# EsauPR/3d-pose-baseline

Measured on AMD Instinct MI355X. Metric: poses/sec at batch 64 (H3.6M 16-joint), higher is better.
Workload: dtype f32; 1 GPU; cfg2 inference: L=1024, 2 residual blocks, BN(eval), keep=1; a step = one batch-64 request (its own 64 poses); 86 requests per persistent p3d_serve launch (5504 rows, whole network per XCD); global_batch=64, linear_size=1024, num_layers=2, parallelism=dp1

## Files before the change

3d-pose-baseline_amd/csrc/p3d.hip:

```cpp
#include <hip/hip_ext.h>
#include "p3d_kernels.h"
#include "p3d_bf16.h"
#include "p3d_eval.h"
#include "p3d_gemm.h"
#include "p3d_data.h"
#include "p3d_clip.h"
#include "p3d_serve.h"
#include "p3d_serve6.h"
#include "p3d_serve_plan.h"
#include "p3d_gemv.h"
#include "p3d_xchg.h"
#include "../../include/p3d.h"

#include <math.h>
#include <stdlib.h>
#include <stdio.h>
#include <string.h>

#include <cstdlib>
#include <mutex>
#include <string>
#include <unordered_set>
#include <vector>

// ... 1074 lines not shown
  }
  if (training) {
    m->serve_ec_dirty = true;
    m->have_cache = true;
    m->x_cached = x;
    m->B_cached = B;
    m->keep = keep_prob;
    m->seed = seed; m->ctr = ctr; m->row_off = row_offset;
    m->ctr_dev = (ctr == P3D_CTR_GLOBAL_STEP) ? &m->dstate->global_step : nullptr;
  }
  return P3D_OK;
}

extern "C" int p3d_forward(p3d_model* m, const float* x, int64_t B, float* y, int32_t training,
                           float keep_prob, uint64_t seed, uint64_t ctr, int64_t row_offset, void* stream) {
  return p3d_forward_ex(m, x, B, y, training, keep_prob, seed, ctr, row_offset, 0, stream);
}

static_assert(kServe6Rows == P3D_SERVE6_ROWS, "p3d_serve_plan.h plans for the slabs p3d_serve.h sizes");
#define SERVE_KERNEL_k_serve(D, NDT, NCM, RT, PAIR) k_serve<D, NDT, 4>
#define SERVE_KERNEL_k_serve5(D, NDT, NCM, RT, PAIR) k_serve5<D, NDT, 2, 2>
#define SERVE_KERNEL_k_serve6(D, NDT, NCM, RT, PAIR) k_serve6<D, NDT, NCM, RT, PAIR>
#define SERVE_KERNEL_k_serve6_rounds(D, NDT, NCM, RT, PAIR) k_serve6_rounds<D, NDT, NCM, RT>
#define SERVE_KERNEL_ROW(KIND, D, NDT, NCM, RT, PAIR) SERVE_KERNEL_##KIND(D, NDT, NCM, RT, PAIR),
static void (*const kServeKernels[])(ServeArgs) = {P3D_SERVE_FORMS(SERVE_KERNEL_ROW)};
#undef SERVE_KERNEL_ROW

#define SERVE_TRY(expr)                                                                                     \
  do {                                                                                                      \
    hipError_t e_ = (expr);                                                                                 \
    if (e_ != hipSuccess) return fail(P3D_ERR_HIP, std::string("p3d_serve: ") + hipGetErrorString(e_)); \
  } while (0)

static const char* serve_shape_error(const p3d_cfg& c, int64_t B) {
  if (B <= 0) return "p3d_serve: batch must be positive";
  if (c.dtype != P3D_DTYPE_F32) return "p3d_serve: fp32 models only";
  if (c.linear_size <= 0 || c.linear_size % 128 != 0 || c.input_size > 64 || c.output_size > 64 ||
      2 * c.num_layers + 2 > P3D_SERVE_MAXL)
    return "p3d_serve: needs linear_size % 128 == 0, input/output size <= 64, <= 7 blocks";
  if ((B + 63) / 64 > 0x7fffffff) return "p3d_serve: too many rows";
  return nullptr;
}

static int serve_alloc(p3d_model* m) {
  const p3d_cfg& c = m->cfg;
  const int L = c.linear_size, U = L / 32, NDT = (c.output_size + 15) / 16;
// ... 49 lines not shown
  a.sync = m->serve_sync; a.err = m->serve_err;
  a.epoch = m->serve_sync + 3 * P3D_SERVE_SYNC_WORDS;
  a.census_extra = m->serve_fault ? 1 : 0;
  a.delay = (m->serve_delay > 0 && (m->serve_calls++ & 1) == 0) ? m->serve_delay : 0;
  a.delay_xcc = m->serve_delay_xcc;
  a.max_groups = m->serve_groups;
  for (size_t l = 0; l < m->layers.size(); ++l) {
    const Layer& ly = m->layers[l];
    ServeLayer& s = a.ly[l];
    s.Wf = m->wpk + ly.wf; s.bias = m->flat[0] + ly.b;
    if (ly.bn) {
      s.gamma = m->flat[0] + ly.gamma; s.beta = m->flat[0] + ly.beta;
      s.mmean = m->moving + ly.mmean; s.mvar = m->moving + ly.mvar;
    }
    s.wsq = c.max_norm ? m->wsq + ly.widx : nullptr;
  }
  if (B != m->serve_B || (t != nullptr) != m->serve_with_loss) {
    const ServeChoice ch = serve_plan(L, c.num_layers, (c.output_size + 15) / 16, m->serve_grid, m->serve_knobs, B,
                                      t != nullptr);
    if (ch.refused) return fail(P3D_ERR_ARG, ch.refused);
    m->serve_choice = ch; m->serve_B = B; m->serve_with_loss = t != nullptr;
  }
  const ServeForm& f = *m->serve_choice.form;
  const bool use6 = f.kind == SK_k_serve6 || f.kind == SK_k_serve6_rounds;
  a.split = m->serve_choice.S;
  a.nb = m->serve_choice.nb;
  a.ecg = m->serve_ecg;
  HP(0);
  hipStreamCaptureStatus cap = hipStreamCaptureStatusNone;
  SERVE_TRY(hipStreamIsCapturing(st, &cap));
  const bool capturing = cap != hipStreamCaptureStatusNone;
  HP(1);

  if (use6 && (m->serve_ec_dirty || capturing)) {
    const int nl = 2 * c.num_layers + 1;
    k_serve_prep<<<(unsigned)((nl * L + 255) / 256), 256, 0, st>>>(a, m->serve_ecg);
    LAUNCH_CHECK("k_serve_prep");
    if (!capturing) m->serve_ec_dirty = false;
  }
  if (use6) {
    a.act = m->serve6_act;
    a.part = nullptr;
  } else {
    a.sync = m->serve_sync + 2 * P3D_SERVE_SYNC_WORDS;
    SERVE_TRY(hipMemsetAsync(a.sync, 0, P3D_SERVE_SYNC_WORDS * sizeof(unsigned), st));
  }
  if (t) {
    a.tgt = t; a.loss = loss;
    a.lpart = m->serve_loss; a.lcnt = (unsigned*)(m->serve_loss + kServeLossTiles);
    if (m->hwait && !f.pair) { a.hflag = m->hflag_dev; a.hseq = m->hwait; m->harmed = true; }
  }
  ProfScope ps(m, "serve");
  HP(2);
  go(ps, kServeKernels[&f - kServeForms], dim3((unsigned)m->serve_grid), dim3(f.kind == SK_k_serve ? 512 : 256), st, a);
  HP(3);
  LAUNCH_CHECK("k_serve");
  return P3D_OK;
}
#undef SERVE_TRY

extern "C" int p3d_serve(p3d_model* m, const float* x, int64_t B, float* y, void* stream) {
  return serve_impl(m, x, B, y, nullptr, nullptr, stream);
}

extern "C" int p3d_serve_mse(p3d_model* m, const float* x, int64_t B, float* y, const float* t, float* loss,
                             void* stream) {
  if (!t || !loss) return fail(P3D_ERR_ARG, "p3d_serve_mse: null argument");
  return serve_impl(m, x, B, y, t, loss, stream);
}

extern "C" int p3d_serve_plan(const p3d_cfg* cfg, int32_t cus, int64_t B, int32_t with_loss, char* name,
                              int64_t name_len, int32_t* shape) {
  if (!cfg || !name || name_len <= 0 || cus < 1) return fail(P3D_ERR_ARG, "p3d_serve_plan: bad argument");
  if (const char* why = serve_shape_error(*cfg, B)) return fail(P3D_ERR_ARG, why);
  const ServeChoice ch = serve_plan(cfg->linear_size, cfg->num_layers, (cfg->output_size + 15) / 16, cus,
                                    serve_knobs_from_env(), B, with_loss != 0);
  if (ch.refused) return fail(P3D_ERR_ARG, ch.refused);
// ... 1071 lines not shown
```

3d-pose-baseline_amd/csrc/p3d_serve6.h:

```cpp
#pragma once
#include "p3d_serve.h"

#ifndef P3D_S6_PIN_ARGS
#define P3D_S6_PIN_ARGS 1
#endif
#ifndef P3D_S6_COMBINE_BATCH
#define P3D_S6_COMBINE_BATCH 1
#endif
#ifndef P3D_S6_OUT_PRE
#define P3D_S6_OUT_PRE 1
#endif
#ifndef P3D_S6_LATE_EPOCH
#define P3D_S6_LATE_EPOCH 1
#endif


#ifdef P3D_TRACE
#define P3D_S6_STAMP(row, k)                                                              \
  do {                                                                                    \
    if (tr6 && (row) && threadIdx.x == 0) {                                               \
      tr6[(k)] = wall_clock64();                                                          \
      tr6[64 + (k)] = __builtin_amdgcn_s_memtime();                                       \
    }                                                                                     \
  } while (0)
#else
#define P3D_S6_STAMP(row, k) do { } while (0)
#endif

__global__ __launch_bounds__(256) void k_serve_prep(ServeArgs p, float* ecg) {
  const int i = blockIdx.x * 256 + threadIdx.x;
  const int L = p.L, nl = 2 * p.nblk + 1;
  if (i >= nl * L) return;
  const int l = i / L, col = i % L, t = col >> 4, j = col & 15;
  const ServeLayer& ly = p.ly[l];
  float inv = 1.f, shift = 0.f;
  if (p.bn) {
    inv = (1.0f / sqrtf(ly.mvar[col] + p.eps)) * ly.gamma[col];
    shift = ly.beta[col] - ly.mmean[col] * inv;
  }
  float* e = ecg + ((int64_t)l * (L >> 4) + t) * 48;
  e[j] = ly.bias[col]; e[16 + j] = inv; e[32 + j] = shift;
  if (col == 0)
    ecg[(int64_t)nl * (L >> 4) * 48 + l] = ly.wsq ? fmaxf(sqrtf(*ly.wsq), 1.0f) : 1.0f;
}

__device__ __forceinline__ int p3d_tile_owner(int t, int n, int T) { return ((t + 1) * n - 1) / T; }

template <int DEPTH, int NDT, int NCM, int RT = 4, bool PAIR = false>
__global__ __launch_bounds__(256) __attribute__((amdgpu_waves_per_eu(1, 1))) void k_serve6(ServeArgs p) {
  constexpr bool ROUNDS = false;
#include "p3d_serve6_body.h"
}

template <int DEPTH, int NDT, int NCM, int RT>
__global__ __launch_bounds__(256) __attribute__((amdgpu_waves_per_eu(1, 1))) void k_serve6_rounds(ServeArgs p) {
  constexpr bool PAIR = true, ROUNDS = true;
#include "p3d_serve6_body.h"
}
```

3d-pose-baseline_amd/csrc/p3d_serve6_body.h:

```cpp
  static_assert(RT >= 1 && RT <= 16, "row tiles per unit");
  static_assert(!PAIR || (NCM == 2 && DEPTH == 4), "the pair form: 2 column tiles per member, a 4-deep ring");
  constexpr int ROWS = 16 * RT;
  constexpr int UMAX = (RT * NCM + 3) / 4;
  constexpr int OCH = RT * NCM < 4 ? RT * NCM : 4;
#ifndef P3D_S6_DA
  constexpr int DA = PAIR ? DEPTH : RT >= 6 ? (DEPTH >= 8 ? 4 : 2) : (NCM >= 7 && DEPTH > 2 ? 2 : DEPTH);
#else
  constexpr int DA = RT >= 6 ? P3D_S6_DA : (NCM >= 7 && DEPTH > 2 ? 2 : DEPTH);
#endif
#ifndef P3D_S6_PD
  constexpr int PD = NCM <= 4 ? 2 : 1;
#else
  constexpr int PD = P3D_S6_PD;
#endif
  static_assert(!PAIR || DA == DEPTH, "the pair form's ring runs on across blocks: every slot holds both operands");
  __shared__ __attribute__((aligned(16))) f32x4 red[(PAIR ? 2 : 1) * 4 * RT * NCM * 64];
  constexpr int ECT = NCM >= 7 ? NCM : 2 * NCM;
  __shared__ __attribute__((aligned(16))) float ec[(P3D_SERVE_MAXL - 1) * ECT * 48];
  __shared__ float ecm[P3D_SERVE_MAXL];
  __shared__ int sh[32];
  const int tid = threadIdx.x, lane = tid & 63, w = __builtin_amdgcn_readfirstlane(tid >> 6);
#if P3D_S6_PIN_ARGS
  asm volatile("" ::"s"(p.split), "s"(p.delay), "s"(p.delay_xcc), "s"(p.census_extra), "s"(p.max_groups),
               "s"(p.nb), "s"(p.L), "s"(p.K0), "s"(p.nblk), "s"(p.M), "s"(p.x), "s"(p.epoch), "s"(p.ecg),
               "s"(p.err), "s"(p.sync), "s"(p.act), "s"(p.ly[0].Wf), "s"(gridDim.x));
#endif
  const int L = p.L, ngL = L >> 4, T = ngL, ngK0 = p.K0 >> 4;
  const int q4 = 4 * (lane >> 4);
  const int S = min(max(p.split, 1), 8);
#ifdef P3D_TRACE
  const unsigned long long t_start = wall_clock64();
  unsigned long long* tr6 = nullptr;
#endif

  const int nxg = (int)(gridDim.x >> 3);
  unsigned xr;
  asm volatile("s_getreg_b32 %0, hwreg(HW_REG_XCC_ID)" : "=s"(xr));
  const int xcc = (int)(xr & 7u), rx = (int)(blockIdx.x >> 3);
  unsigned ep = 0;
  if (tid == 0) {
    if (p.delay > 0 && xcc == p.delay_xcc)
      for (int i = 0; i < p.delay; ++i) __builtin_amdgcn_s_sleep(127);
    const bool bad = (gridDim.x & 7u) != 0u || p.split < 1 || p.split > 8 || p.census_extra;
    sh[0] = (int)(((unsigned)xcc - blockIdx.x) & 7u);
    sh[2] = bad ? 1 : 0;
    sh[4] = 0;
    sh[5] = -1;
    sh[6] = 0;
    if (bad) __hip_atomic_store(p.err, 1, __ATOMIC_RELAXED, __HIP_MEMORY_SCOPE_SYSTEM);
  }
  const int nl_ec = 2 * p.nblk + 1, tot_ec = nl_ec * ECT * 48;
  constexpr int ECN = ((P3D_SERVE_MAXL - 1) * ECT * 48 + 255) / 256;
  auto place = [&](auto cnt, int xcc, int rx, int& r, int& n, int& gid, int& gi, int& ng) {
    const int half = rx % S;
    r = rx / S;
    n = (cnt(xcc) + S - 1 - half) / S;
    gid = xcc * S + half;
    ng = 0;
    gi = 0;
    for (int h = 0; h < S; ++h)
#pragma unroll
      for (int x = 0; x < 8; ++x) {
        const int c = (cnt(x) + S - 1 - h) / S;
        if (c > 0) { if (x == xcc && h == half) gi = ng; ++ng; }
      }
    if (p.max_groups > 0 && ng > p.max_groups) {
      ng = p.max_groups;
      if (gi >= ng) gi = p.nb;
    }
    if ((T + n - 1) / n > ECT) gi = -1;
    if (PAIR && ((T + n - 1) / n > NCM || n > T || (T >> 2) < 3 * DEPTH)) gi = -1;
// ... 5 lines not shown
#pragma unroll
    for (int j = 0; j < (PAIR ? 0 : UMAX); ++j) {
      const int u = min(w + 4 * j, RT * NCM - 1), rt = u / NCM, cc = u % NCM;
      int64_t rowc = (int64_t)gi_ * ROWS + 16 * rt + (lane & 15);
      rowc = rowc < p.M ? (rowc > 0 ? rowc : 0) : p.M - 1;
      const int t = min(max(tlo + (cc < nck ? cc : nck - 1), 0), T - 1);
#pragma unroll
      for (int g = 0; g < 2; ++g) {
        const int gg = min(g, ngK0 - 1);
        xa0[j][g] = *(const f32x4*)(p.x + rowc * p.K0 + 16 * gg + q4);
        wb0[j][g] = *(const f32x4*)(p.ly[0].Wf + ((int64_t)(t * ngK0 + gg) * 64 + lane) * 4);
      }
      if (ngK0 > 2) {
#pragma unroll
        for (int g = 2; g < 4; ++g) {
          const int gg = min(g, ngK0 - 1);
          xa0[j][g] = *(const f32x4*)(p.x + rowc * p.K0 + 16 * gg + q4);
          wb0[j][g] = *(const f32x4*)(p.ly[0].Wf + ((int64_t)(t * ngK0 + gg) * 64 + lane) * 4);
        }
      }
    }
#pragma unroll
    for (int k = 0; k < ECN; ++k) {
      const int idx = tid + 256 * k, idc = idx < tot_ec ? idx : 0;
      const int l = idc / (ECT * 48), rem = idc % (ECT * 48), cs = rem / 48, j = rem % 48;
      const float e = p.ecg[((int64_t)l * T + min(tlo + cs, T - 1)) * 48 + j];
      vec[k] = idx < tot_ec ? e : 0.f;
    }
    const float e = p.ecg[(int64_t)nl_ec * T * 48 + (tid < nl_ec ? tid : 0)];
    wq = tid < nl_ec ? e : 1.f;
  };
  int r, n, gid, gi, ng;
  const bool placeable = (gridDim.x & 7u) == 0u && p.split >= 1 && p.split <= 8;
  place([&](int) { return nxg; }, xcc, rx, r, n, gid, gi, ng);
#if P3D_S6_LATE_EPOCH
  prefetch(gi, (T * r) / n, (T * (r + 1)) / n);
  if (tid == 0 && placeable) ep = __hip_atomic_load(p.epoch + gid, __ATOMIC_RELAXED, __HIP_MEMORY_SCOPE_AGENT);
#else
  if (tid == 0 && placeable) ep = __hip_atomic_load(p.epoch + gid, __ATOMIC_RELAXED, __HIP_MEMORY_SCOPE_AGENT);
  prefetch(gi, (T * r) / n, (T * (r + 1)) / n);
  if (tid == 0) {
    sh[3] = (int)(ep & 1u);
    sh[5] = (placeable && r == 0 && gi >= 0 && gi < p.nb) ? gid : -1;
  }
  __syncthreads();
#endif
#ifdef P3D_TRACE
// ... 49 lines not shown
      const int u = min(w + 4 * j, RT * NCM - 1), rt = u / NCM, cc = u % NCM;
      int64_t rowc = rbase + 16 * rt + (lane & 15);
      rowc = rowc < p.M ? rowc : p.M - 1;
      const int t = c0 + (cc < nck ? cc : nck - 1);
#pragma unroll
      for (int g = 0; g < 2; ++g) {
        const int gg = min(g, ngK0 - 1);
        xa[j][g] = *(const f32x4*)(p.x + rowc * p.K0 + 16 * gg + q4);
        wb[j][g] = *(const f32x4*)(li.Wf + ((int64_t)(t * ngK0 + gg) * 64 + lane) * 4);
      }
      if (ngK0 > 2) {
#pragma unroll
        for (int g = 2; g < 4; ++g) {
          const int gg = min(g, ngK0 - 1);
          xa[j][g] = *(const f32x4*)(p.x + rowc * p.K0 + 16 * gg + q4);
          wb[j][g] = *(const f32x4*)(li.Wf + ((int64_t)(t * ngK0 + gg) * 64 + lane) * 4);
        }
      }
    }
  };
  {
#pragma unroll
    for (int k = 0; k < ECN; ++k)
      if (tid + 256 * k < tot_ec) ec[tid + 256 * k] = vec[k];
    if (tid < nl_ec) ecm[tid] = wq;
    __syncthreads();
  }
  P3D_S6_STAMP(trs, 4);
  auto epi_c = [&](const f32x4& b4, const f32x4& inv4, const f32x4& sh4, f32x4 acc) -> f32x4 {
    f32x4 o;
#pragma unroll
    for (int k = 0; k < 4; ++k) {
      const float z = acc[k] + b4[k];
      o[k] = p3d_relu(p.bn ? z * inv4[k] + sh4[k] : z);
    }
    return o;
  };
  auto epi_t = [&](int l, int cs, f32x4 acc) -> f32x4 {
    const float* e = ec + (l * ECT + cs) * 48 + q4;
    return epi_c(*(const f32x4*)e, *(const f32x4*)(e + 16), *(const f32x4*)(e + 32), acc);
  };
  auto maxnorm_div = [&](int l, f32x4& acc) {
    const float mx = ecm[l];
#pragma unroll
    for (int k = 0; k < 4; ++k) acc[k] = acc[k] / mx;
  };

// ... 73 lines not shown
    }
  };

  const float qnan = __builtin_nanf("");
  constexpr int OGH = 8;
  f32x4 ow0[OGH], ow1[OGH];
  auto out_wpre = [&]() {
    const int oo = (((PAIR ? 2 : 1) * RT * NDT * r) / n) % NDT;
    const __amdgpu_buffer_rsrc_t r4 = p3d_rsrc(lo.Wf);
#pragma unroll
    for (int g = 0; g < OGH; ++g) {
      ow0[g] = __builtin_bit_cast(f32x4, __builtin_amdgcn_raw_buffer_load_b128(r4, ((oo * ngL + gb + min(g, gcount - 1)) * 64 + lane) * 16, 0, 0));
      ow1[g] = __builtin_bit_cast(f32x4, __builtin_amdgcn_raw_buffer_load_b128(r4, ((oo * ngL + gb + min(OGH + g, gcount - 1)) * 64 + lane) * 16, 0, 0));
    }
  };
#ifdef P3D_TRACE
#define P3D_S6_OSTAMP(k)                                                                               \
  do {                                                                                                 \
    if (tid == 0 && blockIdx.x < 1024) g_p3d_trace[21504 + blockIdx.x * 4 + (k)] = wall_clock64();     \
  } while (0)
#else
#define P3D_S6_OSTAMP(k) do { } while (0)
#endif
  auto out_phase = [&](int64_t orow0, int64_t orow1, bool pre) {
    constexpr int OT = RT * NDT, OTT = PAIR ? 2 * OT : OT;
    const int o_lo = (OTT * r) / n, o_hi = (OTT * (r + 1)) / n;
    P3D_S6_OSTAMP(0);
    const __amdgpu_buffer_rsrc_t ryA = p3d_rsrc(act + 3 * slab), r4 = p3d_rsrc(lo.Wf);
    const __amdgpu_buffer_rsrc_t ryB = p3d_rsrc(act + (PAIR ? 7 : 3) * slab);
    for (int c0 = o_lo; c0 < o_hi; c0 += OCH) {
      const int nt = min(OCH, o_hi - c0);
      f32x4 tv = f32x4{0.f, 0.f, 0.f, 0.f};
      if (p.tgt && w < nt) {
        const bool tb = PAIR && c0 + w >= OT;
        tv = p3d_serve_load_tgt<NDT>(p, (tb ? c0 + w - OT : c0 + w) * 64 + lane, tb ? orow1 : orow0);
      }
      f32x4 oacc[OCH];
#pragma unroll
      for (int j = 0; j < OCH; ++j) oacc[j] = f32x4{0.f, 0.f, 0.f, 0.f};
#pragma unroll
      for (int j = 0; j < OCH; ++j) {
        if (j >= nt) break;
        const bool tb = PAIR && c0 + j >= OT;
        const int tile = tb ? c0 + j - OT : c0 + j, ort = tile / NDT, oo = tile % NDT;
        const __amdgpu_buffer_rsrc_t ry = tb ? ryB : ryA;
        constexpr int GH = OGH;
        auto ld_half = [&](int gs, f32x4 (&av)[GH], f32x4 (&wv)[GH], bool wpre) {
#pragma unroll
          for (int g = 0; g < GH; ++g) {
            const int gg = gb + min(gs + g, gcount - 1);
            av[g] = p3d_ld_sc1(ry, ((ort * ngL + gg) * 64 + lane) * 16);
            if (!wpre)
              wv[g] = __builtin_bit_cast(f32x4, __builtin_amdgcn_raw_buffer_load_b128(r4, ((oo * ngL + gg) * 64 + lane) * 16, 0, 0));
          }
        };
        auto mma_half = [&](int gs, const f32x4 (&av)[GH], const f32x4 (&wv)[GH]) {
#pragma unroll
          for (int g = 0; g < GH; ++g) {
            if (gs + g >= gcount) break;
#pragma unroll
            for (int e = 0; e < 4; ++e) oacc[j] = __builtin_amdgcn_mfma_f32_16x16x4f32(av[g][e], wv[g][e], oacc[j], 0, 0, 0);
          }
        };
        for (int g0 = 0; g0 < gcount; g0 += 2 * GH) {
          f32x4 a0[GH], w0[GH], a1[GH], w1[GH];
          const bool wpre = P3D_S6_OUT_PRE && pre && c0 == o_lo && j == 0 && g0 == 0;
          if (wpre) {
#pragma unroll
            for (int g = 0; g < GH; ++g) { w0[g] = ow0[g]; w1[g] = ow1[g]; }
          }
          ld_half(g0, a0, w0, wpre);
          ld_half(g0 + GH, a1, w1, wpre);
          mma_half(g0, a0, w0);
          mma_half(g0 + GH, a1, w1);
        }
      }
#pragma unroll
      for (int j = 0; j < OCH; ++j)
        if (j < nt) red[(w * OCH + j) * 64 + lane] = oacc[j];
      if (c0 == o_lo) P3D_S6_OSTAMP(1);
      __syncthreads();
      if (w < nt) {
        f32x4 sl[4];
#pragma unroll
        for (int k = 0; k < 4; ++k) sl[k] = red[(k * OCH + w) * 64 + lane];
        __builtin_amdgcn_sched_barrier(0);
        f32x4 tot = sl[0];
#pragma unroll
        for (int k = 1; k < 4; ++k) tot += sl[k];
        if (broken) tot = f32x4{qnan, qnan, qnan, qnan};
        const bool tb = PAIR && c0 + w >= OT;
        const int tile = tb ? c0 + w - OT : c0 + w;
        const int64_t orow = tb ? orow1 : orow0;
        const float se = p3d_serve_store_out<NDT>(p, lo, tot, tile * 64 + lane, orow, tv);
        if (p.tgt)
          p3d_serve_loss_tile<!PAIR>(p, se, (orow >> 4) * NDT + tile, ((p.M + 15) >> 4) * NDT);
      }
      if (c0 == o_lo) P3D_S6_OSTAMP(2);
      __syncthreads();
    }
  };

  f32x4 rbp[PD][NCM];
  auto b_prefetch = [&](int layer, int c0) {
    const int nck = min(NCM, t_hi - c0);
#pragma unroll
    for (int cc = 0; cc < NCM; ++cc) {
      const int t = c0 + (cc < nck ? cc : nck - 1);
      const f32x4* pbn = (const f32x4*)p.ly[layer].Wf + ((int64_t)t * ngL + gb) * 64 + lane;
#pragma unroll
      for (int d = 0; d < PD; ++d) rbp[d][cc] = pbn[d * 64];
    }
  };

  if constexpr (!PAIR) {
  int c0b = 0;
  if (gi < p.nb) {
    if (t_lo < t_hi) in_compute(t_lo, xa0, wb0, act);
    P3D_S6_STAMP(trs, 5);
    in_layer((int64_t)gi * ROWS, act, t_lo + NCM);
    P3D_S6_STAMP(trs, 2);
    if (t_lo < t_hi) b_prefetch(1, t_lo);
// ... 216 lines not shown
  const int aoff0 = (gb * 64 + lane) * 16, rstride = ngL * 1024, voff = lane * 16;
  int toff[NCM];
#pragma unroll
  for (int cc = 0; cc < NCM; ++cc) toff[cc] = ((t_lo + (cc < nck ? cc : nck - 1)) * ngL + gb) * 1024;
  f32x4 ra_[DA][RT], rb_[DEPTH][NCM];
  auto ring_load = [&](int layer, const float* A) {
    const __amdgpu_buffer_rsrc_t ra = p3d_rsrc(A), rw = p3d_rsrc(p.ly[layer].Wf);
#pragma unroll
    for (int d = 0; d < DEPTH; ++d) {
      if (d < DA)
#pragma unroll
        for (int t = 0; t < RT; ++t) ra_[d][t] = p3d_ld_sc1(ra, aoff0 + t * rstride + d * 1024);
#pragma unroll
      for (int cc = 0; cc < NCM; ++cc)
        rb_[d][cc] = __builtin_bit_cast(f32x4, __builtin_amdgcn_raw_buffer_load_b128(rw, voff, toff[cc] + d * 1024, 0));
      __builtin_amdgcn_sched_barrier(0);
    }
  };
  int rot = 0;
  int64_t orowA = 0, orowB = 0;
#ifdef P3D_TRACE
  int rnd = 0;
#endif
  if constexpr (ROUNDS) {
    if (gi < p.nb) {
      const int64_t rowA = (int64_t)gi * ROWS, rowB = (int64_t)(gi + ng) * ROWS;
      {
        f32x4 xa[UMAX][4], wa[UMAX][4], xb[UMAX][4], wbb[UMAX][4];
        in_issue(rowA, t_lo, xa, wa);
        in_issue(rowB, t_lo, xb, wbb);
        in_compute(t_lo, xa, wa, act);
        P3D_S6_STAMP(trs, 5);
        group_sync(false, false);
        in_compute(t_lo, xb, wbb, act + 4 * slab);
        P3D_S6_STAMP(trs, 2);
      }
      wait_for(nsync);
      P3D_S6_STAMP(trs, 3);
      {
        const float *A0, *r0;
        float* Y0;
        slabs(0, 0, A0, Y0, r0);
        ring_load(1, A0);
      }
    }
  }
// ... 180 lines not shown
    if (tid == 0 && blockIdx.x < 1024) g_p3d_trace[20480 + blockIdx.x] = wall_clock64();
#endif
    trs = false;
    if constexpr (ROUNDS) {
      rot = rotn;
      orowA = rowA;
      orowB = rowB;
#ifdef P3D_TRACE
      ++rnd;
#endif
    }
  }
  if constexpr (ROUNDS) {
    if (gi < p.nb) {
      const int64_t rowA = orowA, rowB = orowB;
      asm volatile("s_waitcnt vmcnt(0)" ::: "memory");
      post_wave();
      if (P3D_S6_OUT_PRE) out_wpre();
      wait_for(nsync);
      out_phase(rowA, rowB, true);
    }
  }
  }
  if (tid == 0 && sh[5] >= 0)
    __hip_atomic_fetch_add(p.epoch + sh[5], 1u, __ATOMIC_RELAXED, __HIP_MEMORY_SCOPE_AGENT);
  }
```

3d-pose-baseline_amd/csrc/p3d_serve_plan.h:

```cpp
#pragma once
#include <algorithm>
#include <cstdint>
#include <cstdlib>
#include <string>

#define P3D_SERVE_FORMS(X)                                                                      \
  X(k_serve, 2, 1, 0, 4, false) X(k_serve, 2, 2, 0, 4, false) X(k_serve, 2, 3, 0, 4, false)      \
  X(k_serve, 2, 4, 0, 4, false)                                                                 \
  X(k_serve5, 4, 1, 0, 4, false) X(k_serve5, 4, 2, 0, 4, false) X(k_serve5, 4, 3, 0, 4, false)  \
  X(k_serve5, 4, 4, 0, 4, false)                                                                \
  X(k_serve5, 2, 1, 0, 4, false) X(k_serve5, 2, 2, 0, 4, false) X(k_serve5, 2, 3, 0, 4, false)  \
  X(k_serve5, 2, 4, 0, 4, false)                                                                \
  X(k_serve6, 4, 3, 2, 4, false) X(k_serve6, 2, 3, 2, 4, false) X(k_serve6, 4, 3, 4, 4, false)  \
  X(k_serve6, 2, 3, 4, 4, false) X(k_serve6, 4, 3, 7, 4, false) X(k_serve6, 2, 3, 7, 4, false)  \
  X(k_serve6, 2, 3, 8, 4, false)                                                                \
  X(k_serve6, 4, 3, 2, 1, false) X(k_serve6, 4, 3, 2, 2, false) X(k_serve6, 2, 3, 11, 2, false) \
  X(k_serve6, 4, 3, 2, 6, false) X(k_serve6, 4, 3, 2, 8, false) X(k_serve6, 4, 3, 2, 10, false) \
  X(k_serve6, 4, 3, 2, 12, false) X(k_serve6, 4, 3, 2, 16, false)                               \
  X(k_serve6, 4, 3, 2, 5, true) X(k_serve6_rounds, 4, 3, 2, 5, true)

enum ServeKind { SK_k_serve, SK_k_serve5, SK_k_serve6, SK_k_serve6_rounds };

struct ServeForm {
  ServeKind kind;
  int depth, ndt, ncm, rt;
  bool pair;
};

#define P3D_SERVE_FORM_ROW(KIND, DEPTH, NDT, NCM, RT, PAIR) {SK_##KIND, DEPTH, NDT, NCM, RT, PAIR},
constexpr ServeForm kServeForms[] = {P3D_SERVE_FORMS(P3D_SERVE_FORM_ROW)};
#undef P3D_SERVE_FORM_ROW

inline const ServeForm* serve_form_find(ServeKind kind, int depth, int ndt, int ncm, int rt, bool pair) {
  for (const ServeForm& f : kServeForms)
    if (f.kind == kind && f.depth == depth && f.ndt == ndt && f.ncm == ncm && f.rt == rt && f.pair == pair) return &f;
  return nullptr;
}

inline std::string serve_kernel_name(ServeKind kind, int depth, int ndt, int ncm, int rt, bool pair) {
  const std::string dn = std::to_string(depth) + ", " + std::to_string(ndt);
  const std::string cr = ", " + std::to_string(ncm) + ", " + std::to_string(rt);
  switch (kind) {
    case SK_k_serve: return "k_serve<" + dn + ", 4>";
    case SK_k_serve5: return "k_serve5<" + dn + ", 2, 2>";
    case SK_k_serve6_rounds: return "k_serve6_rounds<" + dn + cr + ">";
    default: return "k_serve6<" + dn + cr + (pair ? ", true>" : ">");
  }
}
inline std::string serve_form_name(const ServeForm& f) {
  return serve_kernel_name(f.kind, f.depth, f.ndt, f.ncm, f.rt, f.pair);
}

inline ServeKind serve_fallback_kind(int num_layers) { return num_layers > 0 ? SK_k_serve5 : SK_k_serve; }
inline int serve_fallback_depth(int L, int num_layers) { return num_layers > 0 && (L / 64) % 4 == 0 ? 4 : 2; }

constexpr int kServe6Rows = 4096;
constexpr int64_t kServeLossTiles = kServe6Rows / 16 * 4;

struct ServeKnobs {
  int serve6 = 1;
  int max_nb = 32;
  int split = 0;
  int rt = 0;
  int depth = 2;
  int pair = 1;
  int rounds = 1;
};

inline ServeKnobs serve_knobs_from_env() {
  ServeKnobs k;
  const auto read = [](const char* name, int& v) { if (const char* ev = getenv(name)) v = atoi(ev); };
  read("P3D_SERVE6", k.serve6);
  read("P3D_SERVE6_MAX_NB", k.max_nb);
  read("P3D_SERVE6_SPLIT", k.split);
  read("P3D_SERVE6_RT", k.rt);
  read("P3D_SERVE6_DEPTH", k.depth);
  read("P3D_SERVE6_PAIR", k.pair);
  read("P3D_SERVE6_ROUNDS", k.rounds);
  return k;
}

struct ServeChoice {
  const ServeForm* form = nullptr;
  int S = 0, nb = 0;
  const char* refused = nullptr;
};

struct Serve6Shape { int S = 0, rt = 4, ncm = 0; };

inline Serve6Shape serve6_price(int T, int cus, const ServeKnobs& k, int64_t B) {
  const auto ncm_for = [](int rt, int need) {
    int best = 0;
    for (const ServeForm& f : kServeForms)
      if (f.kind == SK_k_serve6 && !f.pair && f.rt == rt && f.ncm >= need && (!best || f.ncm < best)) best = f.ncm;
    return best;
  };
  static const int rts[] = {4, 2, 1, 6, 8, 10, 12, 16};
  const int cx = std::max(1, cus / 8);
  const double cfix = 4.0;
  Serve6Shape best;
  double bt = 1e30;
// ... 22 lines not shown
  const int T = L / 16;
  ServeChoice c;
  c.nb = (int)((B + 63) / 64);
  if (with_loss && (B + 15) / 16 * NDT > kServeLossTiles) {
    c.refused = "p3d_serve_mse: more 16 x 16 output tiles than the loss partials buffer holds: use p3d_serve + p3d_mse";
    return c;
  }
  const bool long_launch = c.nb > (int64_t)k.max_nb;
  const bool long_pair = long_launch && k.serve6 == 1 && k.rounds && k.pair && !with_loss && num_layers > 0 &&
                         NDT == 3 && L / 64 >= 12 && (L / 64) % 4 == 0 && cus >= 8 &&
                         (T + cus / 8 - 1) / (cus / 8) <= 2 && T >= cus / 8 && (k.split == 0 || k.split == 1) &&
                         (k.rt == 0 || k.rt == 10);
  if (k.serve6 && num_layers > 0 && NDT == 3 && (k.serve6 == 2 || !long_launch || long_pair)) {
    Serve6Shape s;
    if (long_pair) { s.S = 1; s.rt = 10; s.ncm = 2; }
    else s = serve6_price(T, cus, k, B);
    if (s.S > 0) {
      const bool pair = k.pair && s.S == 1 && s.rt == 10 && L / 64 >= 12;
      if (pair) s.rt = 5;
      int depth = ((s.ncm <= 4 || (s.ncm == 7 && k.depth == 4)) && (T / 4) % 4 == 0) ? 4 : 2;
      if (s.rt == 2) depth = s.ncm == 2 ? 4 : 2;
      if (s.rt == 1 || s.rt > 4) depth = 4;
      const bool rounds = pair && long_launch && k.rounds && !with_loss;
      c.form = serve_form_find(rounds ? SK_k_serve6_rounds : SK_k_serve6, depth, NDT, s.ncm, s.rt, pair);
      if (!c.form) { c.refused = "p3d_serve: the planned k_serve6 form is not built"; return c; }
      c.S = s.S;
      c.nb = (int)((B + 16 * s.rt - 1) / (16 * s.rt));
      return c;
    }
  }
  if (with_loss) {
    c.refused = "p3d_serve_mse: no k_serve6 form covers this launch (more than 32 batch-64 steps, "
                "or a model shape k_serve6 is not built for): use p3d_serve + p3d_mse";
    return c;
  }
  c.form = serve_form_find(serve_fallback_kind(num_layers), serve_fallback_depth(L, num_layers), NDT, 0, 4, false);
  if (!c.form) c.refused = "p3d_serve: no serve kernel is built for this many output columns";
  return c;
}
```

Baseline: 11.87 million poses/s.

## Add helper wavefronts to rounds serve kernel for epilogue and input-layer overlap

The persistent rounds kernel now launches 512 threads: four compute waves run the hidden-layer MFMA GEMMs and push partial sums to LDS, while four helper waves do the reduction, BN/bias epilogue, residual add, input layer, output phase and cross-group posting. The two sides hand off through LDS counters with sleep-based spin waits, and the helpers get raised priority. This is meant to take epilogue and sync latency off the critical GEMM waves. The cost is two waves per EU (occupancy 2), so each wave has fewer registers, plus new LDS handshakes that could stall or spill. The old 256-thread form is kept as a w4 variant, selected through an env knob.

```diff
diff --git a/3d-pose-baseline_amd/csrc/p3d.hip b/3d-pose-baseline_amd/csrc/p3d.hip
--- a/3d-pose-baseline_amd/csrc/p3d.hip
+++ b/3d-pose-baseline_amd/csrc/p3d.hip
@@ -1120,6 +1120,7 @@
 #define SERVE_KERNEL_k_serve5(D, NDT, NCM, RT, PAIR) k_serve5<D, NDT, 2, 2>
 #define SERVE_KERNEL_k_serve6(D, NDT, NCM, RT, PAIR) k_serve6<D, NDT, NCM, RT, PAIR>
 #define SERVE_KERNEL_k_serve6_rounds(D, NDT, NCM, RT, PAIR) k_serve6_rounds<D, NDT, NCM, RT>
+#define SERVE_KERNEL_k_serve6_rounds_w4(D, NDT, NCM, RT, PAIR) k_serve6_rounds_w4<D, NDT, NCM, RT>
 #define SERVE_KERNEL_ROW(KIND, D, NDT, NCM, RT, PAIR) SERVE_KERNEL_##KIND(D, NDT, NCM, RT, PAIR),
 static void (*const kServeKernels[])(ServeArgs) = {P3D_SERVE_FORMS(SERVE_KERNEL_ROW)};
 #undef SERVE_KERNEL_ROW
@@ -1215,7 +1216,7 @@
     m->serve_choice = ch; m->serve_B = B; m->serve_with_loss = t != nullptr;
   }
   const ServeForm& f = *m->serve_choice.form;
-  const bool use6 = f.kind == SK_k_serve6 || f.kind == SK_k_serve6_rounds;
+  const bool use6 = serve_kind_is6(f.kind);
   a.split = m->serve_choice.S;
   a.nb = m->serve_choice.nb;
   a.ecg = m->serve_ecg;
@@ -1245,7 +1246,7 @@
   }
   ProfScope ps(m, "serve");
   HP(2);
-  go(ps, kServeKernels[&f - kServeForms], dim3((unsigned)m->serve_grid), dim3(f.kind == SK_k_serve ? 512 : 256), st, a);
+  go(ps, kServeKernels[&f - kServeForms], dim3((unsigned)m->serve_grid), dim3((unsigned)serve_kind_threads(f.kind)), st, a);
   HP(3);
   LAUNCH_CHECK("k_serve");
   return P3D_OK;
diff --git a/3d-pose-baseline_amd/csrc/p3d_serve6.h b/3d-pose-baseline_amd/csrc/p3d_serve6.h
--- a/3d-pose-baseline_amd/csrc/p3d_serve6.h
+++ b/3d-pose-baseline_amd/csrc/p3d_serve6.h
@@ -12,6 +12,12 @@
 #endif
 #ifndef P3D_S6_LATE_EPOCH
 #define P3D_S6_LATE_EPOCH 1
+#endif
+#ifndef P3D_S6_HELPER_NAP
+#define P3D_S6_HELPER_NAP 8
+#endif
+#ifndef P3D_S6_HELPER_PRIO
+#define P3D_S6_HELPER_PRIO 2
 #endif
 
 
@@ -48,12 +54,18 @@
 
 template <int DEPTH, int NDT, int NCM, int RT = 4, bool PAIR = false>
 __global__ __launch_bounds__(256) __attribute__((amdgpu_waves_per_eu(1, 1))) void k_serve6(ServeArgs p) {
-  constexpr bool ROUNDS = false;
+  constexpr bool ROUNDS = false, HELPERS = false;
 #include "p3d_serve6_body.h"
 }
 
 template <int DEPTH, int NDT, int NCM, int RT>
-__global__ __launch_bounds__(256) __attribute__((amdgpu_waves_per_eu(1, 1))) void k_serve6_rounds(ServeArgs p) {
-  constexpr bool PAIR = true, ROUNDS = true;
+__global__ __launch_bounds__(512) __attribute__((amdgpu_waves_per_eu(2, 2))) void k_serve6_rounds(ServeArgs p) {
+  constexpr bool PAIR = true, ROUNDS = true, HELPERS = true;
 #include "p3d_serve6_body.h"
 }
+
+template <int DEPTH, int NDT, int NCM, int RT>
+__global__ __launch_bounds__(256) __attribute__((amdgpu_waves_per_eu(1, 1))) void k_serve6_rounds_w4(ServeArgs p) {
+  constexpr bool PAIR = true, ROUNDS = true, HELPERS = false;
+#include "p3d_serve6_body.h"
+}
diff --git a/3d-pose-baseline_amd/csrc/p3d_serve6_body.h b/3d-pose-baseline_amd/csrc/p3d_serve6_body.h
--- a/3d-pose-baseline_amd/csrc/p3d_serve6_body.h
+++ b/3d-pose-baseline_amd/csrc/p3d_serve6_body.h
@@ -19,7 +19,8 @@
   __shared__ __attribute__((aligned(16))) float ec[(P3D_SERVE_MAXL - 1) * ECT * 48];
   __shared__ float ecm[P3D_SERVE_MAXL];
   __shared__ int sh[32];
-  const int tid = threadIdx.x, lane = tid & 63, w = __builtin_amdgcn_readfirstlane(tid >> 6);
+  const int tid = threadIdx.x, lane = tid & 63, w = __builtin_amdgcn_readfirstlane(HELPERS ? (tid >> 6) & 3 : tid >> 6);
+  const int tidc = HELPERS ? (tid & 255) : tid;
 #if P3D_S6_PIN_ARGS
   asm volatile("" ::"s"(p.split), "s"(p.delay), "s"(p.delay_xcc), "s"(p.census_extra), "s"(p.max_groups),
                "s"(p.nb), "s"(p.L), "s"(p.K0), "s"(p.nblk), "s"(p.M), "s"(p.x), "s"(p.epoch), "s"(p.ecg),
@@ -47,6 +48,11 @@
     sh[4] = 0;
     sh[5] = -1;
     sh[6] = 0;
+    if constexpr (HELPERS) {
+      sh[7] = 0;
+      sh[8] = 0;
+      sh[9] = 0;
+    }
     if (bad) __hip_atomic_store(p.err, 1, __ATOMIC_RELAXED, __HIP_MEMORY_SCOPE_SYSTEM);
   }
   const int nl_ec = 2 * p.nblk + 1, tot_ec = nl_ec * ECT * 48;
@@ -98,7 +104,7 @@
     }
 #pragma unroll
     for (int k = 0; k < ECN; ++k) {
-      const int idx = tid + 256 * k, idc = idx < tot_ec ? idx : 0;
+      const int idx = tidc + 256 * k, idc = idx < tot_ec ? idx : 0;
       const int l = idc / (ECT * 48), rem = idc % (ECT * 48), cs = rem / 48, j = rem % 48;
       const float e = p.ecg[((int64_t)l * T + min(tlo + cs, T - 1)) * 48 + j];
       vec[k] = idx < tot_ec ? e : 0.f;
@@ -194,7 +200,7 @@
   {
 #pragma unroll
     for (int k = 0; k < ECN; ++k)
-      if (tid + 256 * k < tot_ec) ec[tid + 256 * k] = vec[k];
+      if ((!HELPERS || tid < 256) && tidc + 256 * k < tot_ec) ec[tidc + 256 * k] = vec[k];
     if (tid < nl_ec) ecm[tid] = wq;
     __syncthreads();
   }
@@ -314,10 +320,34 @@
 #else
 #define P3D_S6_OSTAMP(k) do { } while (0)
 #endif
+  unsigned hbn = 0;
+  auto hbar = [&]() {
+    hbn += 4;
+    asm volatile("s_waitcnt lgkmcnt(0)" ::: "memory");
+    if (lane == 0) __hip_atomic_fetch_add(&sh[9], 1, __ATOMIC_RELAXED, __HIP_MEMORY_SCOPE_WORKGROUP);
+    for (int spin = 0;; ++spin) {
+      const unsigned v = (unsigned)__builtin_amdgcn_readfirstlane(
+          __hip_atomic_load(&sh[9], __ATOMIC_RELAXED, __HIP_MEMORY_SCOPE_WORKGROUP));
+      if (v >= hbn) break;
+      if (spin > P3D_SERVE_SPIN) {
+        broken = true;
+        sh[4] = 1;
+        if (lane == 0) __hip_atomic_store(p.err, 1, __ATOMIC_RELAXED, __HIP_MEMORY_SCOPE_SYSTEM);
+        break;
+      }
+      __builtin_amdgcn_s_sleep(1);
+    }
+    asm volatile("" ::: "memory");
+  };
   auto out_phase = [&](int64_t orow0, int64_t orow1, bool pre) {
     constexpr int OT = RT * NDT, OTT = PAIR ? 2 * OT : OT;
     const int o_lo = (OTT * r) / n, o_hi = (OTT * (r + 1)) / n;
     P3D_S6_OSTAMP(0);
+    f32x4* const ro = HELPERS ? red + 4 * RT * NCM * 64 : red;
+    auto obar = [&]() {
+      if constexpr (HELPERS) hbar();
+      else __syncthreads();
+    };
     const __amdgpu_buffer_rsrc_t ryA = p3d_rsrc(act + 3 * slab), r4 = p3d_rsrc(lo.Wf);
     const __amdgpu_buffer_rsrc_t ryB = p3d_rsrc(act + (PAIR ? 7 : 3) * slab);
     for (int c0 = o_lo; c0 < o_hi; c0 += OCH) {
@@ -336,7 +366,7 @@
         const bool tb = PAIR && c0 + j >= OT;
         const int tile = tb ? c0 + j - OT : c0 + j, ort = tile / NDT, oo = tile % NDT;
         const __amdgpu_buffer_rsrc_t ry = tb ? ryB : ryA;
-        constexpr int GH = OGH;
+        constexpr int GH = HELPERS ? 4 : OGH;
         auto ld_half = [&](int gs, f32x4 (&av)[GH], f32x4 (&wv)[GH], bool wpre) {
 #pragma unroll
           for (int g = 0; g < GH; ++g) {
@@ -369,13 +399,13 @@
       }
 #pragma unroll
       for (int j = 0; j < OCH; ++j)
-        if (j < nt) red[(w * OCH + j) * 64 + lane] = oacc[j];
+        if (j < nt) ro[(w * OCH + j) * 64 + lane] = oacc[j];
       if (c0 == o_lo) P3D_S6_OSTAMP(1);
-      __syncthreads();
+      obar();
       if (w < nt) {
         f32x4 sl[4];
 #pragma unroll
-        for (int k = 0; k < 4; ++k) sl[k] = red[(k * OCH + w) * 64 + lane];
+        for (int k = 0; k < 4; ++k) sl[k] = ro[(k * OCH + w) * 64 + lane];
         __builtin_amdgcn_sched_barrier(0);
         f32x4 tot = sl[0];
 #pragma unroll
@@ -389,7 +419,7 @@
           p3d_serve_loss_tile<!PAIR>(p, se, (orow >> 4) * NDT + tile, ((p.M + 15) >> 4) * NDT);
       }
       if (c0 == o_lo) P3D_S6_OSTAMP(2);
-      __syncthreads();
+      obar();
     }
   };
 
@@ -652,6 +682,9 @@
 #ifdef P3D_TRACE
   int rnd = 0;
 #endif
+  if constexpr (HELPERS) {
+#include "p3d_serve6_helpers.h"
+  } else {
   if constexpr (ROUNDS) {
     if (gi < p.nb) {
       const int64_t rowA = (int64_t)gi * ROWS, rowB = (int64_t)(gi + ng) * ROWS;
@@ -878,6 +911,7 @@
     }
   }
   }
+  }
   if (tid == 0 && sh[5] >= 0)
     __hip_atomic_fetch_add(p.epoch + sh[5], 1u, __ATOMIC_RELAXED, __HIP_MEMORY_SCOPE_AGENT);
   }
diff --git a/3d-pose-baseline_amd/csrc/p3d_serve6_helpers.h b/3d-pose-baseline_amd/csrc/p3d_serve6_helpers.h
--- /dev/null
+++ b/3d-pose-baseline_amd/csrc/p3d_serve6_helpers.h
@@ -0,0 +1,267 @@
+  const bool helper = __builtin_amdgcn_readfirstlane(tid >> 8) != 0;
+  int qb = 0;
+#if P3D_S6_HELPER_PRIO == 1
+  if (!helper) __builtin_amdgcn_s_setprio(1);
+#elif P3D_S6_HELPER_PRIO == 2
+  if (helper) __builtin_amdgcn_s_setprio(1);
+#endif
+
+  auto lds_wait = [&](int* word, int target, int nap) {
+    for (int spin = 0;; ++spin) {
+      const int v = __builtin_amdgcn_readfirstlane(__hip_atomic_load(word, __ATOMIC_RELAXED, __HIP_MEMORY_SCOPE_WORKGROUP));
+      if (v >= target) break;
+      if (spin > P3D_SERVE_SPIN) {
+        broken = true;
+        sh[4] = 1;
+        if (lane == 0) __hip_atomic_store(p.err, 1, __ATOMIC_RELAXED, __HIP_MEMORY_SCOPE_SYSTEM);
+        break;
+      }
+      if (nap) __builtin_amdgcn_s_sleep(P3D_S6_HELPER_NAP);
+    }
+    asm volatile("" ::: "memory");
+  };
+  auto in_layer_h = [&](int64_t rbase, float* dst) {
+    f32x4 xa[UMAX][2], wb[UMAX][2];
+    const float* xr[UMAX];
+    const float* wr[UMAX];
+#pragma unroll
+    for (int j = 0; j < UMAX; ++j) {
+      const int u = min(w + 4 * j, RT * NCM - 1), rt = u / NCM, cc = u % NCM;
+      int64_t rowc = rbase + 16 * rt + (lane & 15);
+      rowc = rowc < p.M ? rowc : p.M - 1;
+      const int t = t_lo + (cc < nck ? cc : nck - 1);
+      xr[j] = p.x + rowc * p.K0 + q4;
+      wr[j] = li.Wf + ((int64_t)t * ngK0 * 64 + lane) * 4;
+#pragma unroll
+      for (int g = 0; g < 2; ++g) {
+        const int gg = min(g, ngK0 - 1);
+        xa[j][g] = *(const f32x4*)(xr[j] + 16 * gg);
+        wb[j][g] = *(const f32x4*)(wr[j] + gg * 256);
+      }
+    }
+#pragma unroll
+    for (int j = 0; j < UMAX; ++j) {
+      const int u = w + 4 * j, rt = u / NCM, cc = u % NCM;
+      if (u >= RT * NCM || cc >= nck) continue;
+      const int t = t_lo + cc;
+      const float* e = ec + (0 * ECT + (t - t_lo)) * 48 + q4;
+      const f32x4 c0 = *(const f32x4*)e, c1 = *(const f32x4*)(e + 16), c2 = *(const f32x4*)(e + 32);
+      f32x4 acc = f32x4{0.f, 0.f, 0.f, 0.f};
+#pragma unroll
+      for (int g = 0; g < 2; ++g)
+        if (g < ngK0)
+#pragma unroll
+          for (int k = 0; k < 4; ++k) acc = __builtin_amdgcn_mfma_f32_16x16x4f32(wb[j][g][k], xa[j][g][k], acc, 0, 0, 0);
+      if (ngK0 > 2) {
+        f32x4 xh[2], wh[2];
+#pragma unroll
+        for (int g = 0; g < 2; ++g) {
+          const int gg = min(2 + g, ngK0 - 1);
+          xh[g] = *(const f32x4*)(xr[j] + 16 * gg);
+          wh[g] = *(const f32x4*)(wr[j] + gg * 256);
+        }
+#pragma unroll
+        for (int g = 0; g < 2; ++g)
+          if (2 + g < ngK0)
+#pragma unroll
+            for (int k = 0; k < 4; ++k) acc = __builtin_amdgcn_mfma_f32_16x16x4f32(wh[g][k], xh[g][k], acc, 0, 0, 0);
+      }
+      if (wsq_any) maxnorm_div(0, acc);
+      *(f32x4*)(dst + ((int64_t)(rt * ngL + t) * 64 + lane) * 4) = epi_c(c0, c1, c2, acc);
+    }
+  };
+  if (gi < p.nb) {
+    const int64_t rowA = (int64_t)gi * ROWS, rowB = (int64_t)(gi + ng) * ROWS;
+    if (helper) in_layer_h(rowA, act);
+    group_sync(false, false);
+    if (helper) {
+      in_layer_h(rowB, act + 4 * slab);
+      asm volatile("s_waitcnt vmcnt(0)" ::: "memory");
+      post_wave();
+    } else {
+      wait_for(nsync);
+      P3D_S6_STAMP(trs, 3);
+      const float *A0, *r0;
+      float* Y0;
+      slabs(0, 0, A0, Y0, r0);
+      ring_load(1, A0);
+    }
+  }
+  if (!helper) {
+    for (int b = gi; b < p.nb; b += 2 * ng) {
+      const bool has_next = b + 2 * ng < p.nb;
+      const int rotn = (rot + 2 * p.nblk) % 3;
+      for (int s = 0; s < 2 * NH; ++s) {
+        const int ph = (s >> 1) + 1;
+        const ServeLayer& ly = p.ly[ph];
+        const float *A, *res;
+        float* Y;
+        slabs(s, rot, A, Y, res);
+        const __amdgpu_buffer_rsrc_t ra = p3d_rsrc(A), rw = p3d_rsrc(ly.Wf);
+        P3D_S6_STAMP(trs, 8 + 4 * s);
+        P3D_S6_STAMP(rnd == 1 && s < 3, 41 + 8 * s);
+        f32x4 acc[NCM][RT];
+#pragma unroll
+        for (int cc = 0; cc < NCM; ++cc)
+#pragma unroll
+          for (int t = 0; t < RT; ++t) acc[cc][t] = f32x4{0.f, 0.f, 0.f, 0.f};
+        auto mfmas = [&](int d) {
+#pragma unroll
+          for (int e = 0; e < 4; ++e)
+#pragma unroll
+            for (int cc = 0; cc < NCM; ++cc)
+#pragma unroll
+              for (int t = 0; t < RT; ++t)
+                acc[cc][t] = __builtin_amdgcn_mfma_f32_16x16x4f32(rb_[d][cc][e], ra_[d][t][e], acc[cc][t], 0, 0, 0);
+        };
+        constexpr int kSlotLoads = RT + NCM;
+        auto refill = [&](int d, const __amdgpu_buffer_rsrc_t& ra2, const __amdgpu_buffer_rsrc_t& rw2, int g) {
+#pragma unroll
+          for (int t = 0; t < RT; ++t) ra_[d][t] = p3d_ld_sc1(ra2, aoff0 + t * rstride + g * 1024);
+#pragma unroll
+          for (int cc = 0; cc < NCM; ++cc)
+            rb_[d][cc] = __builtin_bit_cast(f32x4, __builtin_amdgcn_raw_buffer_load_b128(rw2, voff, toff[cc] + g * 1024, 0));
+        };
+        auto round = [&](int g0) {
+#pragma unroll
+          for (int d = 0; d < DEPTH; ++d) {
+            mfmas(d);
+            refill(d, ra, rw, g0 + DEPTH + d);
+            __builtin_amdgcn_sched_barrier(0);
+          }
+        };
+        round(0);
+        asm volatile("s_waitcnt vmcnt(%0)\n\ts_nop 5" ::"n"(DEPTH * kSlotLoads) : "memory");
+        ++nsync;
+        __builtin_amdgcn_sched_barrier(0);
+        for (int g0 = DEPTH; g0 < gcount - 2 * DEPTH; g0 += DEPTH) round(g0);
+        const unsigned fl = __hip_atomic_load(flags + m0 + min(lane, cntw - 1), __ATOMIC_RELAXED, __HIP_MEMORY_SCOPE_AGENT);
+        const int rdw = __hip_atomic_load(&sh[8], __ATOMIC_RELAXED, __HIP_MEMORY_SCOPE_WORKGROUP);
+        __builtin_amdgcn_sched_barrier(0);
+        round(gcount - 2 * DEPTH);
+        if (!broken) {
+          if (__any(fl & 0x80000000u)) broken = true;
+          else if (!__all((fl & 0x7fffffffu) >= nsync)) wait_for(nsync);
+        }
+        asm volatile("" ::: "memory");
+        {
+          const bool wrap = has_next && s == 2 * NH - 1;
+          const int sn = wrap ? 0 : min(s + 1, 2 * NH - 1);
+          const float *An, *rn;
+          float* Yn;
+          slabs(sn, wrap ? rotn : rot, An, Yn, rn);
+          const __amdgpu_buffer_rsrc_t ran = p3d_rsrc(An), rwn = p3d_rsrc(p.ly[(sn >> 1) + 1].Wf);
+          __builtin_amdgcn_sched_barrier(0);
+#pragma unroll
+          for (int d = 0; d < DEPTH; ++d) {
+            mfmas(d);
+            refill(d, ran, rwn, d);
+            __builtin_amdgcn_sched_barrier(0);
+          }
+        }
+        P3D_S6_STAMP(trs, 8 + 4 * s + 1);
+        P3D_S6_STAMP(rnd == 1 && s < 3, 42 + 8 * s);
+        if (__builtin_amdgcn_readfirstlane(rdw) < 4 * (qb - 1)) lds_wait(&sh[8], 4 * (qb - 1), 0);
+        f32x4* rd = red + (s & 1) * (4 * RT * NCM * 64);
+#pragma unroll
+        for (int cc = 0; cc < NCM; ++cc)
+#pragma unroll
+          for (int t = 0; t < RT; ++t) rd[((w * RT + t) * NCM + cc) * 64 + lane] = acc[cc][t];
+        if (broken) sh[4] = 1;
+        asm volatile("s_waitcnt lgkmcnt(0)" ::: "memory");
+        if (lane == 0) __hip_atomic_fetch_add(&sh[7], 1, __ATOMIC_RELAXED, __HIP_MEMORY_SCOPE_WORKGROUP);
+        ++qb;
+      }
+#ifdef P3D_TRACE
+      if (trs && tr6 && tid == 0) tr6[8 * (NH + 1)] = wall_clock64();
+      if (tid == 0 && blockIdx.x < 1024) g_p3d_trace[20480 + blockIdx.x] = wall_clock64();
+      ++rnd;
+#endif
+      trs = false;
+      rot = rotn;
+    }
+  } else {
+    for (int b = gi; b < p.nb; b += 2 * ng) {
+      const int64_t rowA = (int64_t)b * ROWS, rowB = (int64_t)(b + ng) * ROWS;
+      const bool has_next = b + 2 * ng < p.nb;
+      const int rotn = (rot + 2 * p.nblk) % 3;
+      f32x4 part[UMAX][4], ce[UMAX][3], rv[UMAX];
+      for (int s = 0; s < 2 * NH; ++s) {
+        const int php = (s >> 1) + 1;
+        const float *Ap, *resp;
+        float* Yp;
+        slabs(s, rot, Ap, Yp, resp);
+        const __amdgpu_buffer_rsrc_t rr = p3d_rsrc(resp ? resp : Ap);
+#pragma unroll
+        for (int j = 0; j < UMAX; ++j) {
+          const int u = min(w + 4 * j, RT * NCM - 1), rt = u / NCM, cc = u % NCM;
+          const int t = t_lo + (cc < nck ? cc : nck - 1);
+          rv[j] = p3d_ld_sc1(rr, (int)(((int64_t)(rt * ngL + t) * 64 + lane) * 16));
+        }
+        if (has_next && s >= 2 * NH - 2)
+          in_layer_h(((s & 1) ? rowB : rowA) + (int64_t)2 * ng * ROWS, act + ((s & 1) * 4 + rotn) * slab);
+        lds_wait(&sh[7], 4 * (qb + 1), 1);
+        broken = broken || sh[4] != 0;
+        {
+          const f32x4* rdp = red + (s & 1) * (4 * RT * NCM * 64);
+#pragma unroll
+          for (int j = 0; j < UMAX; ++j) {
+            const int u = min(w + 4 * j, RT * NCM - 1), rt = u / NCM, cc = u % NCM;
+#pragma unroll
+            for (int k = 0; k < 4; ++k) part[j][k] = rdp[((k * RT + rt) * NCM + cc) * 64 + lane];
+            const int t = t_lo + (cc < nck ? cc : nck - 1);
+            const float* e = ec + (php * ECT + (t - t_lo)) * 48 + q4;
+#pragma unroll
+            for (int k = 0; k < 3; ++k) ce[j][k] = *(const f32x4*)(e + 16 * k);
+          }
+        }
+        const bool outs = b != gi && s == 1;
+        asm volatile("s_waitcnt lgkmcnt(0)" ::: "memory");
+        if (!outs && lane == 0) __hip_atomic_fetch_add(&sh[8], 1, __ATOMIC_RELAXED, __HIP_MEMORY_SCOPE_WORKGROUP);
+        {
+          f32x4 sacc[UMAX];
+#pragma unroll
+          for (int j = 0; j < UMAX; ++j) {
+            sacc[j] = part[j][0];
+#pragma unroll
+            for (int k = 1; k < 4; ++k) sacc[j] += part[j][k];
+          }
+          if (wsq_any)
+#pragma unroll
+            for (int j = 0; j < UMAX; ++j) maxnorm_div(php, sacc[j]);
+#pragma unroll
+          for (int j = 0; j < UMAX; ++j) {
+            const int u = min(w + 4 * j, RT * NCM - 1), rt = u / NCM, cc = u % NCM;
+            const int t = t_lo + (cc < nck ? cc : nck - 1);
+            f32x4 yv = epi_c(ce[j][0], ce[j][1], ce[j][2], sacc[j]);
+            if (resp) yv += rv[j];
+            *(f32x4*)(Yp + ((int64_t)(rt * ngL + t) * 64 + lane) * 4) = yv;
+          }
+        }
+        const bool post_first = outs && NH >= 4;
+        if (post_first) {
+          asm volatile("s_waitcnt vmcnt(0)" ::: "memory");
+          post_wave();
+        }
+        if (outs) {
+          wait_for(nsync - (post_first ? 2 : 1));
+          hbar();
+          out_phase(orowA, orowB, false);
+          if (lane == 0) __hip_atomic_fetch_add(&sh[8], 1, __ATOMIC_RELAXED, __HIP_MEMORY_SCOPE_WORKGROUP);
+        }
+        if (!post_first) {
+          asm volatile("s_waitcnt vmcnt(0)" ::: "memory");
+          post_wave();
+        }
+        ++qb;
+      }
+      rot = rotn;
+      orowA = rowA;
+      orowB = rowB;
+    }
+    if (gi < p.nb) {
+      wait_for(nsync);
+      hbar();
+      out_phase(orowA, orowB, false);
+    }
+  }
diff --git a/3d-pose-baseline_amd/csrc/p3d_serve_plan.h b/3d-pose-baseline_amd/csrc/p3d_serve_plan.h
--- a/3d-pose-baseline_amd/csrc/p3d_serve_plan.h
+++ b/3d-pose-baseline_amd/csrc/p3d_serve_plan.h
@@ -17,9 +17,12 @@
   X(k_serve6, 4, 3, 2, 1, false) X(k_serve6, 4, 3, 2, 2, false) X(k_serve6, 2, 3, 11, 2, false) \
   X(k_serve6, 4, 3, 2, 6, false) X(k_serve6, 4, 3, 2, 8, false) X(k_serve6, 4, 3, 2, 10, false) \
   X(k_serve6, 4, 3, 2, 12, false) X(k_serve6, 4, 3, 2, 16, false)                               \
-  X(k_serve6, 4, 3, 2, 5, true) X(k_serve6_rounds, 4, 3, 2, 5, true)
+  X(k_serve6, 4, 3, 2, 5, true) X(k_serve6_rounds, 4, 3, 2, 5, true)                             \
+  X(k_serve6_rounds_w4, 4, 3, 2, 5, true)
 
-enum ServeKind { SK_k_serve, SK_k_serve5, SK_k_serve6, SK_k_serve6_rounds };
+enum ServeKind { SK_k_serve, SK_k_serve5, SK_k_serve6, SK_k_serve6_rounds, SK_k_serve6_rounds_w4 };
+inline bool serve_kind_is6(ServeKind k) { return k == SK_k_serve6 || k == SK_k_serve6_rounds || k == SK_k_serve6_rounds_w4; }
+inline int serve_kind_threads(ServeKind k) { return k == SK_k_serve || k == SK_k_serve6_rounds ? 512 : 256; }
 
 struct ServeForm {
   ServeKind kind;
@@ -44,6 +47,7 @@
     case SK_k_serve: return "k_serve<" + dn + ", 4>";
     case SK_k_serve5: return "k_serve5<" + dn + ", 2, 2>";
     case SK_k_serve6_rounds: return "k_serve6_rounds<" + dn + cr + ">";
+    case SK_k_serve6_rounds_w4: return "k_serve6_rounds_w4<" + dn + cr + ">";
     default: return "k_serve6<" + dn + cr + (pair ? ", true>" : ">");
   }
 }
@@ -65,6 +69,7 @@
   int depth = 2;
   int pair = 1;
   int rounds = 1;
+  int helpers = 1;
 };
 
 inline ServeKnobs serve_knobs_from_env() {
@@ -77,6 +82,7 @@
   read("P3D_SERVE6_DEPTH", k.depth);
   read("P3D_SERVE6_PAIR", k.pair);
   read("P3D_SERVE6_ROUNDS", k.rounds);
+  read("P3D_SERVE6_HELPERS", k.helpers);
   return k;
 }
 
@@ -145,7 +151,8 @@
       if (s.rt == 2) depth = s.ncm == 2 ? 4 : 2;
       if (s.rt == 1 || s.rt > 4) depth = 4;
       const bool rounds = pair && long_launch && k.rounds && !with_loss;
-      c.form = serve_form_find(rounds ? SK_k_serve6_rounds : SK_k_serve6, depth, NDT, s.ncm, s.rt, pair);
+      const ServeKind kind = !rounds ? SK_k_serve6 : k.helpers ? SK_k_serve6_rounds : SK_k_serve6_rounds_w4;
+      c.form = serve_form_find(kind, depth, NDT, s.ncm, s.rt, pair);
       if (!c.form) { c.refused = "p3d_serve: the planned k_serve6 form is not built"; return c; }
       c.S = s.S;
       c.nb = (int)((B + 16 * s.rt - 1) / (16 * s.rt));
```

After: 12.31 million poses/s, median of 6. +3.7%, better.
